# zzuiekongning/MGDT-YOLO

Measured on AMD Instinct MI355X. Metric: images/sec @640x640 bs=32 per GPU, detection forward + NMS (whole job: 1 GPU(s)), higher is better.
Workload: dtype bf16; 1 GPU; mspa_c2f_gd_yolov8-n (MSPA-C2f + GD neck + Detect, nc=80) 640x640 inference, batch 32/GPU: forward + decode + NMS(conf 0.25, iou 0.7), hipGraph replay, 4 batches in flight (one captured graph per resident batch, replayed round-robin on 4 streams); global_batch=32, parallelism=replicas x1 (batch-sharded, no data-path collective), rccl_ranks=1, input=bfloat16 NCHW images, 8 different batches resident in HBM (600 MiB) cycled, detections_last_step=9600, weights=seeded random init (no checkpoints offline), batches_in_flight=4

## Files before the change

### include/mgdt.h

```cpp
#ifndef MGDT_H
#define MGDT_H
#include <stddef.h>
#include <stdint.h>

#ifdef __cplusplus
extern "C" {
#endif

typedef void* mgdt_stream;

typedef enum { MGDT_OK = 0, MGDT_BAD_SHAPE = -1, MGDT_BAD_DTYPE = -2, MGDT_LAUNCH_FAIL = -3, MGDT_BAD_ARG = -4,
               MGDT_WORKSPACE = -5 } mgdt_status;
typedef enum { MGDT_F32 = 0, MGDT_BF16 = 1, MGDT_U8 = 2  } mgdt_dtype;
typedef enum { MGDT_ACT_NONE = 0, MGDT_ACT_SILU = 1, MGDT_ACT_RELU = 2, MGDT_ACT_GELU = 3 } mgdt_act;

typedef struct {
  void* p;
  int32_t n, h, w, c;
  int64_t sn, sh, sw, sc;
} mgdt_view;

const char* mgdt_last_error(void);
const char* mgdt_version(void);

// ... 33 lines not shown
size_t mgdt_cnx_mlp_packed_bytes(int c, int dtype);
int mgdt_cnx_mlp_pack(const float* w1, const float* b1, const float* w2, const float* b2, int c, void* packed, int dtype, mgdt_stream s);
size_t mgdt_cnx_mlp_workspace_bytes(int n, int h, int w, int c);
int mgdt_cnx_mlp_fwd(const mgdt_view* t, const mgdt_view* res, const void* packed, const float* gamma, const float* beta, void* ws,
                     const mgdt_view* y, int dtype, mgdt_stream s);

int mgdt_cnx_block_supported(int n, int h, int w, int c, int dtype);
size_t mgdt_cnx_block_workspace_bytes(int n, int h, int w, int c);
int mgdt_cnx_block_geometry(int h, int w, int c, int* out);
int mgdt_cnx_block_fwd(const mgdt_view* x, const float* dw_w49c, const float* dw_b, const float* ln_w, const float* ln_b, float eps, const void* packed,
                       const float* gamma, const float* beta, const void* tail_w, const float* tail_b, int tail_act, void* ws, size_t ws_bytes,
                       const mgdt_view* y, int dtype, mgdt_stream s);

size_t mgdt_stem2_packed_bytes(void);
int mgdt_stem2_pack(const float* w_folded, void* packed, mgdt_stream s);
int mgdt_stem2_fwd(const mgdt_view* x, int x_dtype, const void* packed0, const float* bias0, const void* packed1, const float* bias1,
                   const mgdt_view* y, mgdt_stream s);
int mgdt_stem2_geometry(int n, int h, int w, int cu_count, int* out);
int mgdt_stem2_route(const mgdt_view* x, int x_dtype, const mgdt_view* y, int cu_count, int* out);

int mgdt_detect_tail_supported(int c2, int c3, int nc, int reg_max, int dtype);
int mgdt_detect_tail_fwd(const mgdt_view* tb, const mgdt_view* tc, const void* wb, const float* bb, const void* wc, const float* bc, int nc,
                         float stride, int a_off, int a_total, const mgdt_view* feat, float* y, unsigned long long* best_keys,
                         const void* wb3, const float* bb3, mgdt_stream s);
int mgdt_detect_tail_aug_fwd(const mgdt_view* tb, const mgdt_view* tc, const void* wb, const float* bb, const void* wc, const float* bc, int nc,
                             float stride, int a_off, int a_total, const mgdt_view* feat, float* y, unsigned long long* best_keys,
                             const void* wb3, const float* bb3, float aug_scale, int aug_flip, float aug_img_w, mgdt_stream s);

int mgdt_scale_img_fwd(const mgdt_view* x, int x_dtype, int flip, int hs, int ws, float pad, const mgdt_view* y, int y_dtype, mgdt_stream s);

int mgdt_csp_block_supported(int mode, int cin, int cout, int wd, int nbtl, int h, int w, int dtype);
int mgdt_csp_block_tiles(int mode, int n, int cin, int cout, int wd, int nbtl, int h, int w, int* geom8);
int mgdt_csp_block_fwd(int mode, const mgdt_view* x, const void* front, const float* front_bias, const void* const* mid,
                       const float* const* mid_bias, int nbtl, int shortcut, const void* back, const float* back_bias, int wd, int act,
                       const mgdt_view* y, float* pool, int dtype, mgdt_stream s);

size_t mgdt_pw_chain_packed_bytes(int wd, int dtype);
int mgdt_pw_chain_pack(int idx, const float* w_oi, const float* conv_bias, const float* bn_gamma, const float* bn_beta, const float* bn_mean,
                       const float* bn_var, float bn_eps, int wd, int dtype, void* packed, mgdt_stream s);
int mgdt_pw_chain3_fwd(const mgdt_view* x, const void* packed, int wd, int act, const mgdt_view* y, int dtype, mgdt_stream s);

int mgdt_conv1x1_inject_supported(int cin, int cout, int h, int w, int hg, int wg, int dtype);
int mgdt_conv1x1_inject_fwd(const mgdt_view* x, const void* packed_w, const float* bias, const mgdt_view* ga, const mgdt_view* gf,
                            const mgdt_view* y, int dtype, mgdt_stream s);

int mgdt_conv1x1_inject_conv_supported(int cin, int cmid, int cout2, int h, int w, int hg, int wg, int dtype);
int mgdt_conv1x1_inject_conv_fwd(const mgdt_view* x, const void* packed_w, const float* bias, const mgdt_view* ga, const mgdt_view* gf,
                                 const mgdt_view* gsrc, const void* packed_wg, const float* bias_g, int cmid,
                                 const void* packed_w2, const float* bias2, int act2, const mgdt_view* y2, int dtype, mgdt_stream s);

int mgdt_laf_fuse_supported(int c0, int oc, int oc2, int h, int w, int h2, int w2, int act1, int act2, int dtype);
int mgdt_laf_fuse_fwd(const mgdt_view* p0, const mgdt_view* x1, const mgdt_view* x2, const void* packed_w1, const float* bias1, int act1,
                      const void* packed_w2, const float* bias2, int act2, const mgdt_view* y, int dtype, mgdt_stream s);

size_t mgdt_groupnorm_workspace_bytes(int n, int c);
int mgdt_groupnorm_fwd(const mgdt_view* x, const float* gamma, const float* beta, int groups, float eps, int act, void* ws, const mgdt_view* y,
                       int dtype, mgdt_stream s);
int mgdt_tood_layer_attn_fwd(const float* sums, int n, int c, int hw, const float* w1, const float* b1, const float* w2, const float* b2, int hid,
                             int stacked, float* scale, mgdt_stream s);
int mgdt_dcnv2_fwd(const mgdt_view* x, const mgdt_view* offset_mask, const float* w_gemm, const float* bias, const mgdt_view* y, int dtype,
                   mgdt_stream s);
int mgdt_dcnv2_mfma_fwd(const mgdt_view* x, const mgdt_view* offset_mask, const void* packed_w, const mgdt_view* y, int dtype, mgdt_stream s);
int mgdt_pixel_gate_fwd(const mgdt_view* x, const mgdt_view* gate, const mgdt_view* y, int dtype, mgdt_stream s);

int mgdt_conv_pack_direct(const float* w_oihw, const float* conv_bias, const float* bn_gamma, const float* bn_beta,
                          const float* bn_mean, const float* bn_var, float bn_eps, int cin_g, int cout, int k,
                          float* w_out, float* bias_out, mgdt_stream s);
int mgdt_conv2d_direct_fwd(const mgdt_view* x, int x_dtype, const float* w_gemm, const float* bias, int k, int stride,
                           int groups, int act, const mgdt_view* y, int dtype, mgdt_stream s);
enum { MGDT_DIRECT_STEM = 0, MGDT_DIRECT_GENERIC = 1, MGDT_DIRECT_REFUSED = 2 };
int mgdt_conv2d_direct_route(const mgdt_view* x, int x_dtype, const mgdt_view* y, int dtype, int k, int stride, int groups, int* out);

#define MGDT_SPR_SPLITS 16
int mgdt_spr_pool_fwd(const mgdt_view* x, float* pooled, int dtype, mgdt_stream s);
int mgdt_spr_attn_fwd(const float* pooled, const float* fc1_w, const float* fc1_b, const float* fc2_w,
                      const float* fc2_b, int n, int c, int groups, int h, int w, int softmax, float* attn, mgdt_stream s);
int mgdt_scale_channels_fwd(const mgdt_view* x, const float* attn, const mgdt_view* y, int dtype, mgdt_stream s);
int mgdt_spr_attn_scale_fwd(const float* pooled, int nsplit, int tiles_x, int tiles_y, const float* fc1_w, const float* fc1_b, const float* fc2_w, const float* fc2_b, int groups,
                            const mgdt_view* x, const mgdt_view* y, const mgdt_view* pool_a, const mgdt_view* pool_b, int dtype, mgdt_stream s);

int mgdt_sppf_pool_fwd(const mgdt_view* x, const mgdt_view* y1, const mgdt_view* y2, const mgdt_view* y3, int dtype,
                       mgdt_stream s);

int mgdt_adaptive_avgpool_fwd(const mgdt_view* x, const mgdt_view* y, int dtype, mgdt_stream s);
int mgdt_bilinear_fwd(const mgdt_view* x, const mgdt_view* y, int dtype, mgdt_stream s);
int mgdt_nearest_fwd(const mgdt_view* x, const mgdt_view* y, int dtype, mgdt_stream s);
int mgdt_copy_fwd(const mgdt_view* x, int x_dtype, const mgdt_view* y, int y_dtype, mgdt_stream s);
int mgdt_image_pad4_fwd(const mgdt_view* x, int x_dtype, const mgdt_view* y, int y_dtype, mgdt_stream s);

int mgdt_space_to_depth2_channels(int c, int y_dtype);
int mgdt_conv_pack_stem6(const float* w6, const float* conv_bias, const float* bn_gamma, const float* bn_beta, const float* bn_mean, const float* bn_var,
                         float bn_eps, int c6, int cout, int dtype, void* packed_out, float* bias_out, mgdt_stream s);
int mgdt_space_to_depth2_fwd(const mgdt_view* x, int x_dtype, const mgdt_view* y, int y_dtype, mgdt_stream s);
int mgdt_stem6_wgrad_unpack(const float* dw3, int cout, int cin, int cp, float* dw6, mgdt_stream s);

#define MGDT_GRN_SPLITS 8
int mgdt_dwconv7_ln_fwd(const mgdt_view* x, const float* dw_w, const float* dw_b, const float* ln_w, const float* ln_b,
                        float eps, const mgdt_view* y, int dtype, mgdt_stream s);
int mgdt_grn_stats_fwd(const mgdt_view* t, const float* gamma, float* ws, float* scale, int dtype, mgdt_stream s);
enum { MGDT_DW_ROW8 = 0, MGDT_DW_ROW10 = 1, MGDT_DW_GENERIC = 2 };
int mgdt_dwconv7_ln_route(int n, int h, int w, int c, int dtype, int* out);

int mgdt_inject_fwd(const mgdt_view* local, const mgdt_view* ga, const mgdt_view* gf, const mgdt_view* y, int dtype,
                    mgdt_stream s);

int mgdt_detect_decode_fwd(const mgdt_view* feat, int reg_max, int nc, float stride, int a_off, int a_total, float* y,
// ... 227 lines not shown
```

### mgdt_yolo_amd/_lib.py

```python
import ctypes as C
import os

_HERE = os.path.dirname(os.path.abspath(__file__))
LIB_PATH = os.environ.get('MGDT_LIB') or os.path.join(_HERE, 'csrc', 'libmgdt_hip.so')

F32, BF16 = 0, 1
ACT_NONE, ACT_SILU, ACT_RELU, ACT_GELU = 0, 1, 2, 3
SPR_SPLITS = 16
GRN_SPLITS = 8


class View(C.Structure):
    _fields_ = [('p', C.c_void_p), ('n', C.c_int32), ('h', C.c_int32), ('w', C.c_int32), ('c', C.c_int32),
                ('sn', C.c_int64), ('sh', C.c_int64), ('sw', C.c_int64), ('sc', C.c_int64)]


VP = C.POINTER(View)
_vp, _i, _f, _sz, _l = C.c_void_p, C.c_int, C.c_float, C.c_size_t, C.c_long

class PackDesc(C.Structure):
    _fields_ = [('w', C.c_void_p), ('conv_bias', C.c_void_p), ('bn_gamma', C.c_void_p), ('bn_beta', C.c_void_p), ('bn_mean', C.c_void_p), ('bn_var', C.c_void_p),
                ('bn_eps', C.c_float), ('cin', C.c_int32), ('cout', C.c_int32), ('k', C.c_int32), ('dtype', C.c_int32), ('mode', C.c_int32),
                ('packed', C.c_void_p), ('bias_out', C.c_void_p)]

# ... 10 lines not shown
ROUTE_X2, ROUTE_IN_SCALE, ROUTE_IN_SHIFT, ROUTE_R1, ROUTE_R2, ROUTE_FP8 = 1, 2, 4, 8, 16, 32
ROUTE_IGEMM, ROUTE_LDS3X3 = 0, 1
DIRECT_STEM, DIRECT_GENERIC, DIRECT_REFUSED = 0, 1, 2

PROTOTYPES = {
    'mgdt_last_error': (C.c_char_p, []),
    'mgdt_version': (C.c_char_p, []),
    'mgdt_conv_packed_bytes': (_sz, [_i, _i, _i, _i]),
    'mgdt_conv_pack': (_i, [_vp, _vp, _vp, _vp, _vp, _vp, _f, _i, _i, _i, _i, _vp, _vp, _vp]),
    'mgdt_conv2d_fwd': (_i, [VP, VP, _vp, _vp, _vp, _vp, _i, _i, _i, VP, VP, VP, _i, _vp]),
    'mgdt_conv_packed_bytes_fp8': (_sz, [_i, _i, _i]),
    'mgdt_conv_pack_fp8': (_i, [_vp, _vp, _vp, _vp, _vp, _vp, _f, _i, _i, _i, _f, _vp, _vp, _vp, _vp]),
    'mgdt_conv2d_fp8_fwd': (_i, [VP, VP, _vp, _vp, _vp, _vp, _vp, _f, _i, _i, _i, VP, VP, VP, _vp]),
    'mgdt_conv2d_route': (_i, [VP, VP, _i, _i, _i, _i, _i, C.POINTER(ConvRoute)]),
    'mgdt_conv_pack_batch': (_i, [_vp, _i, _vp]),
    'mgdt_conv2d_phase_fwd': (_i, [VP, _vp, _vp, _i, VP, VP, VP, _i, _vp]),
    'mgdt_conv_wgrad_splits': (_i, [_i, _i, _i]),
    'mgdt_wgrad_final_batch': (_i, [_vp, _i, _vp]),
    'mgdt_conv_pack_dgrad': (_i, [_vp, _i, _i, _i, _i, _i, _vp, _vp, _vp]),
    'mgdt_conv_pack_direct': (_i, [_vp, _vp, _vp, _vp, _vp, _vp, _f, _i, _i, _i, _vp, _vp, _vp]),
    'mgdt_conv2d_direct_fwd': (_i, [VP, _i, _vp, _vp, _i, _i, _i, _i, VP, _i, _vp]),
    'mgdt_conv2d_direct_route': (_i, [VP, _i, VP, _i, _i, _i, _i, C.POINTER(C.c_int)]),
    'mgdt_spr_pool_fwd': (_i, [VP, _vp, _i, _vp]),
    'mgdt_spr_attn_fwd': (_i, [_vp, _vp, _vp, _vp, _vp, _i, _i, _i, _i, _i, _i, _vp, _vp]),
    'mgdt_scale_channels_fwd': (_i, [VP, _vp, VP, _i, _vp]),
    'mgdt_sppf_pool_fwd': (_i, [VP, VP, VP, VP, _i, _vp]),
    'mgdt_adaptive_avgpool_fwd': (_i, [VP, VP, _i, _vp]),
    'mgdt_bilinear_fwd': (_i, [VP, VP, _i, _vp]),
    'mgdt_nearest_fwd': (_i, [VP, VP, _i, _vp]),
    'mgdt_copy_fwd': (_i, [VP, _i, VP, _i, _vp]),
    'mgdt_image_pad4_fwd': (_i, [VP, _i, VP, _i, _vp]),
    'mgdt_space_to_depth2_channels': (_i, [_i, _i]),
    'mgdt_space_to_depth2_fwd': (_i, [VP, _i, VP, _i, _vp]),
    'mgdt_conv_pack_stem6': (_i, [_vp, _vp, _vp, _vp, _vp, _vp, _f, _i, _i, _i, _vp, _vp, _vp]),
    'mgdt_stem6_wgrad_unpack': (_i, [_vp, _i, _i, _i, _vp, _vp]),
    'mgdt_dwconv7_ln_fwd': (_i, [VP, _vp, _vp, _vp, _vp, _f, VP, _i, _vp]),
    'mgdt_cnx_mlp_packed_bytes': (_sz, [_i, _i]),
    'mgdt_cnx_mlp_pack': (_i, [_vp, _vp, _vp, _vp, _i, _vp, _i, _vp]),
    'mgdt_cnx_mlp_workspace_bytes': (_sz, [_i, _i, _i, _i]),
    'mgdt_cnx_mlp_fwd': (_i, [VP, VP, _vp, _vp, _vp, _vp, VP, _i, _vp]),
    'mgdt_cnx_block_supported': (_i, [_i, _i, _i, _i, _i]),
    'mgdt_cnx_block_workspace_bytes': (_sz, [_i, _i, _i, _i]),
    'mgdt_cnx_block_geometry': (_i, [_i, _i, _i, C.POINTER(C.c_int)]),
    'mgdt_cnx_block_fwd': (_i, [VP, _vp, _vp, _vp, _vp, _f, _vp, _vp, _vp, _vp, _vp, _i, _vp, _sz, VP, _i, _vp]),
    'mgdt_pw_chain_packed_bytes': (_sz, [_i, _i]),
    'mgdt_pw_chain_pack': (_i, [_i, _vp, _vp, _vp, _vp, _vp, _vp, _f, _i, _i, _vp, _vp]),
    'mgdt_pw_chain3_fwd': (_i, [VP, _vp, _i, _i, VP, _i, _vp]),
    'mgdt_conv1x1_inject_supported': (_i, [_i, _i, _i, _i, _i, _i, _i]),
    'mgdt_conv1x1_inject_fwd': (_i, [VP, _vp, _vp, VP, VP, VP, _i, _vp]),
    'mgdt_conv1x1_inject_conv_supported': (_i, [_i, _i, _i, _i, _i, _i, _i, _i]),
    'mgdt_conv1x1_inject_conv_fwd': (_i, [VP, _vp, _vp, VP, VP, VP, _vp, _vp, _i, _vp, _vp, _i, VP, _i, _vp]),
    'mgdt_laf_fuse_supported': (_i, [_i, _i, _i, _i, _i, _i, _i, _i, _i, _i]),
    'mgdt_laf_fuse_fwd': (_i, [VP, VP, VP, _vp, _vp, _i, _vp, _vp, _i, VP, _i, _vp]),
    'mgdt_spr_attn_scale_fwd': (_i, [_vp, _i, _i, _i, _vp, _vp, _vp, _vp, _i, VP, VP, VP, VP, _i, _vp]),
    'mgdt_stem2_packed_bytes': (_sz, []),
    'mgdt_stem2_pack': (_i, [_vp, _vp, _vp]),
    'mgdt_stem2_fwd': (_i, [VP, _i, _vp, _vp, _vp, _vp, VP, _vp]),
    'mgdt_stem2_geometry': (_i, [_i, _i, _i, _i, C.POINTER(C.c_int)]),
    'mgdt_stem2_route': (_i, [VP, _i, VP, _i, C.POINTER(C.c_int)]),
    'mgdt_detect_tail_supported': (_i, [_i, _i, _i, _i, _i]),
    'mgdt_detect_tail_fwd': (_i, [VP, VP, _vp, _vp, _vp, _vp, _i, _f, _i, _i, VP, _vp, _vp, _vp, _vp, _vp]),
    'mgdt_detect_tail_aug_fwd': (_i, [VP, VP, _vp, _vp, _vp, _vp, _i, _f, _i, _i, VP, _vp, _vp, _vp, _vp, _f, _i, _f, _vp]),
    'mgdt_scale_img_fwd': (_i, [VP, _i, _i, _i, _i, _f, VP, _i, _vp]),
    'mgdt_csp_block_supported': (_i, [_i, _i, _i, _i, _i, _i, _i, _i]),
    'mgdt_csp_block_tiles': (_i, [_i, _i, _i, _i, _i, _i, _i, _i, _vp]),
    'mgdt_csp_block_fwd': (_i, [_i, VP, _vp, _vp, _vp, _vp, _i, _i, _vp, _vp, _i, _i, VP, _vp, _i, _vp]),
    'mgdt_groupnorm_workspace_bytes': (_sz, [_i, _i]),
    'mgdt_groupnorm_fwd': (_i, [VP, _vp, _vp, _i, _f, _i, _vp, VP, _i, _vp]),
    'mgdt_tood_layer_attn_fwd': (_i, [_vp, _i, _i, _i, _vp, _vp, _vp, _vp, _i, _i, _vp, _vp]),
    'mgdt_dcnv2_fwd': (_i, [VP, VP, _vp, _vp, VP, _i, _vp]),
    'mgdt_dcnv2_mfma_fwd': (_i, [VP, VP, _vp, VP, _i, _vp]),
    'mgdt_pixel_gate_fwd': (_i, [VP, VP, VP, _i, _vp]),
    'mgdt_gn_affine_workspace_bytes': (_sz, [_i, _i, _i]),
    'mgdt_gn_affine': (_i, [VP, _vp, _vp, _i, _f, _vp, _vp, _vp, _vp, _vp, _i, _vp]),
    'mgdt_nc_affine_act_bwd': (_i, [VP, VP, _vp, _vp, _i, VP, _i, _vp]),
    'mgdt_gn_act_grad': (_i, [VP, VP, _vp, _vp, _vp, _i, _i, VP, _i, _vp]),
    'mgdt_gn_bwd_workspace_bytes': (_sz, [_i, _i]),
    'mgdt_gn_bwd_coef': (_i, [VP, VP, _vp, _vp, _i, _vp, _vp, _vp, _vp, _vp, _i, _vp, _i, _vp]),
    'mgdt_nc_axpby': (_i, [VP, _vp, VP, _vp, _vp, VP, _i, _vp]),
    'mgdt_pixel_gate_bwd': (_i, [VP, VP, VP, VP, VP, _i, _vp]),
    'mgdt_tood_layer_attn_bwd_workspace_bytes': (_sz, [_i, _i, _i, _i]),
    'mgdt_tood_layer_attn_bwd': (_i, [_vp, _vp, _i, _i, _i, _vp, _vp, _vp, _vp, _i, _i, _vp, _vp, _vp, _vp, _vp, _i, _vp, _vp]),
    'mgdt_dcn_im2col': (_i, [VP, VP, VP, _i, _vp]),
    'mgdt_dcn_col2im_bwd': (_i, [VP, VP, VP, _vp, VP, _i, _vp]),
    'mgdt_val_match_fwd': (_i, [_vp, _vp, _i, _i, _vp, _vp, _i, _vp, _i, _vp, _vp]),
    'mgdt_grn_stats_fwd': (_i, [VP, _vp, _vp, _vp, _i, _vp]),
    'mgdt_dwconv7_ln_route': (_i, [_i, _i, _i, _i, _i, C.POINTER(C.c_int)]),
    'mgdt_inject_fwd': (_i, [VP, VP, VP, VP, _i, _vp]),
    'mgdt_detect_decode_fwd': (_i, [VP, _i, _i, _f, _i, _i, _vp, _i, _vp]),
    'mgdt_detect_decode_aug_fwd': (_i, [VP, _i, _i, _f, _i, _i, _vp, _vp, _f, _i, _f, _i, _vp]),
    'mgdt_detect_loss_workspace_bytes': (_sz, [_i, _i, _i]),
    'mgdt_detect_loss_fwd': (_i, [_vp, _vp, _i, _i, _i, _vp, _i, _i, _f, _f, _f, _vp, _vp, _vp, _vp, _vp, _sz, _i, _vp]),
    'mgdt_detect_loss_fwd_dev': (_i, [_vp, _vp, _i, _i, _i, _vp, _i, _vp, _f, _f, _f, _vp, _vp, _vp, _vp, _vp, _sz, _i, _vp]),
    'mgdt_detect_loss_bwd': (_i, [_vp, _vp, _vp, _i, _i, _i, _vp, _i, _f, _f, _f, _f, _vp, _vp, _sz, _i, _vp]),
    'mgdt_reduce_workspace_bytes': (_sz, [_i]),
    'mgdt_bn_stats_fwd': (_i, [VP, _f, _f, _vp, _vp, _vp, _vp, _vp, _i, _vp]),
    'mgdt_bn_act_fwd': (_i, [VP, _vp, _vp, _vp, _vp, _i, VP, VP, VP, _i, _vp]),
    'mgdt_bn_act_bwd': (_i, [VP, VP, _vp, _vp, _vp, _vp, _i, _vp, _vp, VP, _vp, _i, _vp]),
    'mgdt_conv_dgrad': (_i, [VP, _vp, _i, _i, VP, _i, _i, _vp]),
    'mgdt_gconv_dgrad': (_i, [VP, _vp, _i, _i, _i, VP, _i, _i, _vp]),
    'mgdt_gconv_wgrad_workspace_bytes': (_sz, [_i, _i, _i, _i]),
    'mgdt_gconv_wgrad': (_i, [VP, VP, _i, _i, _i, _vp, _i, _vp, _i, _vp]),
    'mgdt_conv_wgrad_workspace_bytes': (_sz, [_i, _i, _i]),
    'mgdt_conv_wgrad': (_i, [VP, VP, VP, _i, _i, _vp, _vp, _i, _vp, _i, _vp]),
    'mgdt_add_fwd': (_i, [VP, VP, VP, _i, _vp]),
    'mgdt_maxpool5_bwd': (_i, [VP, VP, _vp, _i, _vp]),
# ... 106 lines not shown
```

### mgdt_yolo_amd/nn/modules/block.py

```python
import torch
import torch.nn as nn

from ... import ops
from .conv import Conv, HipModule, act_code
from .convnextv2 import ConvNeXtV2_Block
from .spr_module import SPRModule

__all__ = ('DFL', 'SPP', 'SPPF', 'C2f', 'C3', 'MSPA_C2f', 'Bottleneck', 'SimFusion_4in', 'SimFusion_3in', 'IFM', 'h_sigmoid',
           'InjectionMultiSum_Auto_pool', 'Upsample', 'Proto')


def _plain_block(first, last, bottlenecks):
    def conv_ok(c, k):
        return (isinstance(c, Conv) and c.plain_affine() and c.conv.kernel_size == (k, k) and c.conv.stride == (1, 1) and c.conv.groups == 1
                and act_code(c.act) == a0)
    try:
        a0 = act_code(first.act)
    except RuntimeError:
        return False
    if a0 != ops.ACT_SILU:
        return False
    if not (conv_ok(first, 1) and conv_ok(last, 1)) or len(bottlenecks) == 0:
        return False
    return all(isinstance(m, Bottleneck) and conv_ok(m.cv1, 3) and conv_ok(m.cv2, 3) and m.add == bottlenecks[0].add
# ... 214 lines not shown
                   and c.conv.out_channels == self.inwidth and act_code(c.act) == act_code(cs[0].act) for c in cs)

    def _packed_chain(self, dtype):
        cs = list(self.convs)[:3]
        tens = [t for c in cs for t in c.affine_tensors()]
        return self._cached(('chain', dtype), tens, lambda: ops.PackedPwChain([(c.conv.weight, c.conv.bias, c.bn_tuple()) for c in cs], dtype))

    def backward(self, g):
        out, attn, part, xshape = self._ctx.pop()
        wd, s, n = self.inwidth, self.nums, self.btnk_nums
        at = self.attention
        dattn = ops.nc_reduce(g, out)
        prms = (at.fc1.weight, at.fc1.bias, at.fc2.weight, at.fc2.bias)
        gb = [ops.grad_buf(p) for p in prms]
        chained = all(t.is_contiguous() and t.dtype == torch.float32 for t in gb) and all(
            a.untyped_storage().data_ptr() == b.untyped_storage().data_ptr() and a.storage_offset() + a.numel() == b.storage_offset() for a, b in zip(gb, gb[1:]))
        pg_out = gb[0].new_empty(0).set_(gb[0].untyped_storage(), gb[0].storage_offset(), (sum(t.numel() for t in gb),)) if chained else None
        gout, pg = ops.spr_bwd(g, part, attn, dattn, at.fc1.weight, at.fc1.bias, at.fc2.weight, at.fc2.bias, s, out=pg_out)
        if not chained:
            o = 0
            for prm, t in zip(prms, gb):
                t.copy_(pg[o:o + t.numel()].view_as(prm))
                o += t.numel()
        gcat = self.convs[s - 1].backward(gout)
        gx = ops.new_act(xshape[0], xshape[1], xshape[2], xshape[3], g.dtype, g.device)
        sl = lambda t, i: t[:, i * wd:(i + 1) * wd]
        for j in reversed(range(n)):
            if j > 0:
                self.bottleneck[j].backward(sl(gcat, s - 1 + j), acc_into=sl(gcat, s - 2 + j))
                continue
            gin = self.bottleneck[j].backward(sl(gcat, s - 1 + j))
            dst = sl(gcat, s - 2 + j)
            ops.add(dst, gin, out=dst)
            ops.copy(gin, sl(gx, s - 1))
        for i in reversed(range(1, s - 1)):
            gi = self.convs[i].backward(sl(gcat, i), dx_out=sl(gx, i))
            dst = sl(gcat, i - 1)
            ops.add(dst, gi, out=dst)
        self.convs[0].backward(sl(gcat, 0), dx_out=sl(gx, 0))
        return gx


class SPPF(HipModule):

    def __init__(self, c1, c2, k=5):
        super().__init__()
        if k != 5:
            raise RuntimeError('SPPF: k=5 is what the YAMLs use and what the fused pooling kernel implements')
        c_ = c1 // 2
        self.cv1 = Conv(c1, c_, 1, 1)
        self.cv2 = Conv(c_ * 4, c2, 1, 1)
        self.m = nn.MaxPool2d(kernel_size=k, stride=1, padding=k // 2)

    def forward(self, x):
        b, _, h, w = x.shape
        c_ = self.cv1.conv.out_channels
        train = self.training and hasattr(self.cv1, 'bn')
        cat = ops.new_act(b, 4 * c_, h, w, self.cv1.out_dtype(x), x.device)
        (self.cv1.train_fwd if train else self.cv1.run)(x, out=cat[:, :c_])
        ops.sppf_pools(cat[:, :c_], cat[:, c_:2 * c_], cat[:, 2 * c_:3 * c_], cat[:, 3 * c_:])
        if train:
            self._cat = cat if ops.ctx_enabled() else None
        return (self.cv2.train_fwd if train else self.cv2.run)(cat)

    def backward(self, g):
        c_ = self.cv1.conv.out_channels
        cat, self._cat = self._cat, None
        gcat = self.cv2.backward(g)
        sl = lambda t, i: t[:, i * c_:(i + 1) * c_]
        g2 = ops.add(sl(gcat, 2), ops.maxpool5_bwd(sl(cat, 2), sl(gcat, 3)))
        g1 = ops.add(sl(gcat, 1), ops.maxpool5_bwd(sl(cat, 1), g2))
        g0 = ops.add(sl(gcat, 0), ops.maxpool5_bwd(sl(cat, 0), g1))
        return self.cv1.backward(g0)


class SPP(SPPF):

    def __init__(self, c1, c2, k=(5, 9, 13)):
        if tuple(k) != (5, 9, 13):
            raise RuntimeError(f'SPP: k=(5, 9, 13) is what the YAMLs use and what the pooling kernels implement, got {tuple(k)}')
        super().__init__(c1, c2, 5)
        self.m = nn.ModuleList([nn.MaxPool2d(kernel_size=x, stride=1, padding=x // 2) for x in k])

    def backward(self, g):
        c_ = self.cv1.conv.out_channels
        cat, self._cat = self._cat, None
        gcat = self.cv2.backward(g)
        sl = lambda t, i: t[:, i * c_:(i + 1) * c_]
        g0 = ops.add(sl(gcat, 0), ops.spp_pool_bwd(sl(cat, 0), sl(gcat, 1), sl(gcat, 2), sl(gcat, 3)))
        return self.cv1.backward(g0)


class Proto(HipModule):

    def __init__(self, c1, c_=256, c2=32):
        super().__init__()
        self.cv1 = Conv(c1, c_, k=3)
        self.upsample = nn.ConvTranspose2d(c_, c_, 2, 2, 0, bias=True)
        self.cv2 = Conv(c_, c_, k=3)
        self.cv3 = Conv(c_, c2)

    def run_upsample(self, x):
        up = self.upsample
        ops.check_deconv2x2(up.kernel_size, up.stride, up.padding, up.groups, up.output_padding, up.dilation)
        if up.bias is None:
            raise RuntimeError('Proto.upsample is built with its bias (block.py:63)')
        dt = self.out_dtype(x)
        pk = self._cached(('deconv', dt), [up.weight, up.bias], lambda: ops.PackedDeconv2x2(up.weight, up.bias, dt))
        return ops.deconv2x2(x, pk)

# ... 270 lines not shown
```

### mgdt_yolo_amd/ops.py

```python
import ctypes as C
import os

import numpy as np
import torch

from . import _lib as L
from ._lib import ACT_GELU, ACT_NONE, ACT_RELU, ACT_SILU, BF16, F32, View

U8 = 2
_DT = {torch.float32: F32, torch.bfloat16: BF16}


def dtype_code(dt):
    try:
        return _DT[dt]
    except KeyError:
        raise RuntimeError(f'mgdt_yolo_amd computes in float32 or bfloat16, not {dt}') from None


def _need_gpu(t):
    if not t.is_cuda:
        raise RuntimeError('mgdt_yolo_amd runs on MI355X (HIP) only: got a CPU tensor and there is no CPU/PyTorch fallback')


# ... 652 lines not shown


def conv1x1_inject_conv_supported(x, cmid, cout2, ga, dtype):
    return bool(FUSED_INJECT and FUSED_INJECT_CONV and x.dtype == dtype and ga.dtype == dtype and is_nhwc(x) and is_nhwc(ga) and
                L.lib().mgdt_conv1x1_inject_conv_supported(x.shape[1], cmid, cout2, x.shape[2], x.shape[3], ga.shape[2], ga.shape[3], dtype_code(dtype)))


def conv1x1_inject_conv(x, pk, ga, gf, pk2, act2, out, gsrc=None, pkg=None):
    b, _, h, w = x.shape
    _same(x, ga, gf, gsrc, out)
    if _PROF is not None:
        _META['conv1x1_inject_conv_fwd'] = dict(shape=(b, pk.cin, h, w, pk2.cout, 1, 1), flops=2.0 * b * h * w * (pk.cout * pk.cin + pk2.cout * pk2.cin),
                                                bytes=float(b * h * w * (pk.cin + pk2.cout) * x.element_size() + (2 * ga.numel() * ga.element_size() if gsrc is None else gsrc.numel() * 2)))
    _launch('conv1x1_inject_conv_fwd', 'mgdt_conv1x1_inject_conv_fwd', vp(x), ptr(pk.w), ptr(pk.bias), vp(ga), vp(gf), vp(gsrc), None if pkg is None else ptr(pkg.w),
            None if pkg is None else ptr(pkg.bias), pk.cout, ptr(pk2.w), ptr(pk2.bias), int(act2), vp(out), dtype_code(pk.dtype), stream())
    return out


FUSED_INJECT_CONV = True
FUSED_INJECT_GCONV = True


def conv1x1_inject(x, pk, ga, gf, out=None):
    b, _, h, w = x.shape
    if out is None:
        out = new_act(b, pk.cout, h, w, pk.dtype, x.device)
    if _PROF is not None:
        _META['conv1x1_inject_fwd'] = dict(shape=(b, pk.cin, h, w, pk.cout, 1, 1), flops=2.0 * b * h * w * pk.cout * pk.cin,
                                           bytes=float(b * h * w * (pk.cin + pk.cout) * x.element_size() + 2 * ga.numel() * ga.element_size()))
    _launch('conv1x1_inject_fwd', 'mgdt_conv1x1_inject_fwd', vp(x), ptr(pk.w), ptr(pk.bias), vp(ga), vp(gf), vp(out), dtype_code(pk.dtype), stream())
    return out


FUSED_LAF = True


def laf_fuse_supported(p0, x1, x2, oc2, act1, act2, dtype):
    return bool(FUSED_LAF and p0.dtype == dtype and x1.dtype == dtype and x2.dtype == dtype and is_nhwc(p0) and is_nhwc(x1) and is_nhwc(x2) and
                x2.shape[1] == x1.shape[1] and p0.shape[0] == x1.shape[0] == x2.shape[0] and p0.shape[2:] == x1.shape[2:] and
                all(t.stride(0) % 8 == 0 and t.stride(2) % 8 == 0 and t.stride(3) % 8 == 0 and t.data_ptr() % 16 == 0 for t in (p0, x1, x2)) and
                L.lib().mgdt_laf_fuse_supported(p0.shape[1], x1.shape[1], oc2, x1.shape[2], x1.shape[3], x2.shape[2], x2.shape[3], int(act1), int(act2),
                                                dtype_code(dtype)))


def laf_fuse(p0, x1, x2, pk1, act1, pk2, act2, out=None):
    b, oc, h, w = x1.shape
    if out is None:
        out = new_act(b, pk2.cout, h, w, pk2.dtype, x1.device)
    _same(p0, x1, x2, out)
    if _PROF is not None:
        _META['laf_fuse_fwd'] = dict(shape=(b, pk1.cin, h, w, pk2.cout, 1, 1), flops=2.0 * b * h * w * (pk1.cout * pk1.cin + pk2.cout * pk2.cin),
                                     bytes=float((b * h * w * (pk1.cin + oc + pk2.cout) + x2.numel()) * x1.element_size()))
    _launch('laf_fuse_fwd', 'mgdt_laf_fuse_fwd', vp(p0), vp(x1), vp(x2), ptr(pk1.w), ptr(pk1.bias), int(act1), ptr(pk2.w), ptr(pk2.bias), int(act2), vp(out),
            dtype_code(pk2.dtype), stream())
    return out


def groupnorm(x, gamma, beta, groups, eps, act, out=None):
    b, c = x.shape[:2]
    out = like(x) if out is None else out
    ws = torch.empty(L.lib().mgdt_groupnorm_workspace_bytes(b, c), dtype=torch.uint8, device=x.device)
    _launch('groupnorm_fwd', 'mgdt_groupnorm_fwd', vp(x), ptr(gamma), ptr(beta), groups, float(eps), act, ptr(ws), vp(out), dtype_code(x.dtype), stream())
    return out


def tood_layer_attn(feat, w1, b1, w2, b2, stacked, sums=None):
    b, c, h, w = feat.shape
    sums = nc_reduce(feat) if sums is None else sums
    scale = torch.empty(b, c, dtype=torch.float32, device=feat.device)
    _launch('tood_layer_attn_fwd', 'mgdt_tood_layer_attn_fwd', ptr(sums), b, c, h * w, ptr(w1), ptr(b1), ptr(w2), ptr(b2), w1.shape[0], stacked, ptr(scale), stream())
    return scale


def dcnv2(x, offset_mask, w_gemm, bias, cout):
    b, _, h, w = x.shape
    out = new_act(b, cout, h, w, x.dtype, x.device)
    _launch('dcnv2_fwd', 'mgdt_dcnv2_fwd', vp(x), vp(offset_mask), ptr(w_gemm), ptr(bias), vp(out), dtype_code(x.dtype), stream())
    return out


def dcnv2_mfma(x, offset_mask, pk, out=None):
    b, _, h, w = x.shape
    out = new_act(b, pk.cout, h, w, x.dtype, x.device) if out is None else out
    _same(x, offset_mask, out)
    _launch('dcnv2_mfma_fwd', 'mgdt_dcnv2_mfma_fwd', vp(x), vp(offset_mask), ptr(pk.w), vp(out), dtype_code(x.dtype), stream())
    return out


def pixel_gate(x, gate, out=None):
    out = like(x) if out is None else out
    _launch('pixel_gate_fwd', 'mgdt_pixel_gate_fwd', vp(x), vp(gate), vp(out), dtype_code(x.dtype), stream())
    return out


def _gn_affine(y, gamma, beta, groups, eps):
    b, c, h, w = y.shape
    dev = y.device
    A, B = torch.empty(b, c, dtype=torch.float32, device=dev), torch.empty(b, c, dtype=torch.float32, device=dev)
    mean, rstd = torch.empty(b, groups, dtype=torch.float32, device=dev), torch.empty(b, groups, dtype=torch.float32, device=dev)
    ws = torch.empty(L.lib().mgdt_gn_affine_workspace_bytes(b, c, groups), dtype=torch.uint8, device=dev)
    _launch('gn_affine', 'mgdt_gn_affine', vp(y), ptr(gamma), ptr(beta), groups, float(eps), ptr(mean), ptr(rstd), ptr(A), ptr(B), ptr(ws), dtype_code(y.dtype), stream())
    return A, B, mean, rstd, ws[ws.numel() - b * groups * 16:].view(torch.float64).view(b, groups, 2)


def gn_affine(y, gamma, beta, groups, eps):
    return _gn_affine(y, gamma, beta, groups, eps)[:4]
# ... 1631 lines not shown
```

Before: 42410 images/sec.

## Fuse SPPF cv1, cascaded max-pools and cv2 into one LDS-resident kernel

Adds a HIP kernel that runs the whole SPPF block per spatial tile with a 6-pixel halo. It computes cv1 with MFMA into LDS, applies the three cascaded 5x5 max-pools as separable row/column passes in LDS using an order-preserving bf16 key, and accumulates cv2 over the four concat slices before writing only the final output. The aim is to remove the HBM round trips for the 4*c_ concat tensor and the separate pool and conv launches. In exchange, halo pixels are recomputed for every tile and LDS use is large, which limits how many workgroups fit per CU.

After: 43210 images/sec (median of 6 runs). +1.9%, better.

```diff
diff --git a/include/mgdt.h b/include/mgdt.h
--- a/include/mgdt.h
+++ b/include/mgdt.h
@@ -109,6 +109,10 @@
 int mgdt_laf_fuse_supported(int c0, int oc, int oc2, int h, int w, int h2, int w2, int act1, int act2, int dtype);
 int mgdt_laf_fuse_fwd(const mgdt_view* p0, const mgdt_view* x1, const mgdt_view* x2, const void* packed_w1, const float* bias1, int act1,
                       const void* packed_w2, const float* bias2, int act2, const mgdt_view* y, int dtype, mgdt_stream s);
+
+int mgdt_sppf_fuse_supported(int c1, int cm, int c2, int h, int w, int act1, int act2, int dtype);
+int mgdt_sppf_fuse_fwd(const mgdt_view* x, const void* packed_w1, const float* bias1, int act1, const void* packed_w2, const float* bias2, int act2,
+                       const mgdt_view* y, int dtype, mgdt_stream s);
 
 size_t mgdt_groupnorm_workspace_bytes(int n, int c);
 int mgdt_groupnorm_fwd(const mgdt_view* x, const float* gamma, const float* beta, int groups, float eps, int act, void* ws, const mgdt_view* y,
diff --git a/mgdt_yolo_amd/_lib.py b/mgdt_yolo_amd/_lib.py
--- a/mgdt_yolo_amd/_lib.py
+++ b/mgdt_yolo_amd/_lib.py
@@ -86,6 +86,8 @@
     'mgdt_conv1x1_inject_conv_fwd': (_i, [VP, _vp, _vp, VP, VP, VP, _vp, _vp, _i, _vp, _vp, _i, VP, _i, _vp]),
     'mgdt_laf_fuse_supported': (_i, [_i, _i, _i, _i, _i, _i, _i, _i, _i, _i]),
     'mgdt_laf_fuse_fwd': (_i, [VP, VP, VP, _vp, _vp, _i, _vp, _vp, _i, VP, _i, _vp]),
+    'mgdt_sppf_fuse_supported': (_i, [_i, _i, _i, _i, _i, _i, _i, _i]),
+    'mgdt_sppf_fuse_fwd': (_i, [VP, _vp, _vp, _i, _vp, _vp, _i, VP, _i, _vp]),
     'mgdt_spr_attn_scale_fwd': (_i, [_vp, _i, _i, _i, _vp, _vp, _vp, _vp, _i, VP, VP, VP, VP, _i, _vp]),
     'mgdt_stem2_packed_bytes': (_sz, []),
     'mgdt_stem2_pack': (_i, [_vp, _vp, _vp]),
diff --git a/mgdt_yolo_amd/csrc/sppf_fused.hip b/mgdt_yolo_amd/csrc/sppf_fused.hip
--- /dev/null
+++ b/mgdt_yolo_amd/csrc/sppf_fused.hip
@@ -0,0 +1,309 @@
+#include <algorithm>
+
+#include "conv_igemm_kernel.h"
+
+struct SppfArgs {
+  const char* x; int xsn, xsh, xsw; uint32_t x_bytes;
+  const char* y; int ysn, ysh, ysw; uint32_t y_bytes;
+  const char* w1; const float* b1; const char* w2; const float* b2;
+  int H, W, T, tiles_x, tiles_img, act1, act2;
+  int a_bytes;
+  unsigned long long* dbg;
+};
+
+constexpr int SPPF_THREADS = 512, SPPF_CPAD = 8;
+constexpr int SPPF_TILES[] = {10, 8, 6, 5, 4, 3, 2, 1};
+constexpr int SPPF_STATIC = 2048;
+constexpr int SPPF_LDS = 160 * 1024 - SPPF_STATIC;
+
+typedef __attribute__((ext_vector_type(2))) float sppf_f32x2;
+typedef __attribute__((ext_vector_type(2))) __bf16 sppf_bf16x2;
+typedef __attribute__((ext_vector_type(8))) short sppf_i16x8;
+typedef __attribute__((ext_vector_type(4))) unsigned int sppf_u32x4;
+typedef __attribute__((__vector_size__(2 * sizeof(unsigned int)))) unsigned int sppf_u32x2v;
+__device__ __forceinline__ uint32_t sppf_pk_bf16(float lo, float hi) {
+  return __builtin_bit_cast(uint32_t, __builtin_convertvector(sppf_f32x2{lo, hi}, sppf_bf16x2));
+}
+__device__ __forceinline__ uint32_t sppf_key(uint32_t v) { return v ^ (((v >> 15) & 0x00010001u) * 0x7fffu); }
+__device__ __forceinline__ sppf_u32x4 sppf_key4(sppf_u32x4 v) { return sppf_u32x4{sppf_key(v[0]), sppf_key(v[1]), sppf_key(v[2]), sppf_key(v[3])}; }
+__device__ __forceinline__ sppf_u32x4 sppf_kmax(sppf_u32x4 p, sppf_u32x4 q) {
+  return __builtin_bit_cast(sppf_u32x4, __builtin_elementwise_max(__builtin_bit_cast(sppf_i16x8, p), __builtin_bit_cast(sppf_i16x8, q)));
+}
+__device__ __forceinline__ float sppf_nan_pos(float v) { return v != v ? __uint_as_float(0x7fc00000u) : v; }
+__device__ __forceinline__ int sppf_clamp(int v, int hi) { return min(max(v, 0), hi); }
+
+template <int KC1, int NB2>
+__global__ __launch_bounds__(SPPF_THREADS) void sppf_fuse_kernel(const SppfArgs a) {
+  typedef bf16x8 frag;
+  constexpr int NB1 = KC1, KCM = KC1 / 2, CQ = 2 * KC1;
+  constexpr int RS = (NB1 * 16 + SPPF_CPAD) * 2;
+  constexpr int W1V = KC1 * NB1 * 64;
+  constexpr int CW = NB2 % 4 == 0 ? 4 : 2, NBW = NB2 / CW;
+  constexpr int PW = 8 / CW, MT2 = (7 + PW - 1) / PW;
+  static_assert((NB1 + NB2) * 16 * sizeof(float) <= SPPF_STATIC, "the bias vectors outgrow their share of the 160 KiB");
+  static_assert(KC1 % 2 == 0 && MT2 * PW >= 7, "whole K chunks per concat slot; seven pixel groups of a 10 x 10 tile");
+  extern __shared__ __attribute__((aligned(16))) char sppf_sm[];
+  __shared__ __attribute__((aligned(16))) float bl1[NB1 * 16];
+  __shared__ __attribute__((aligned(16))) float bl2[NB2 * 16];
+  char* const A = sppf_sm;
+  char* const B = sppf_sm + a.a_bytes;
+  const int tid = threadIdx.x, lane = tid & 63;
+  const int wave = __builtin_amdgcn_readfirstlane(tid >> 6);
+  const int r = lane & 15, g = lane >> 4;
+  unsigned long long* const dbgw = (a.dbg && tid == 0) ? a.dbg + (size_t)blockIdx.x * 8 : nullptr;
+  if (dbgw) dbgw[0] = wall_clock64();
+
+  const int n = (int)blockIdx.x / a.tiles_img, tile = (int)blockIdx.x - n * a.tiles_img;
+  const int tyi = tile / a.tiles_x, txi = tile - tyi * a.tiles_x;
+  const int H = a.H, W = a.W;
+  const int y0 = tyi * a.T, x0 = txi * a.T, th = min(a.T, H - y0), tw = min(a.T, W - x0);
+  const int ry0 = max(y0 - 6, 0), ry1 = min(y0 + th + 6, H), rx0 = max(x0 - 6, 0), rx1 = min(x0 + tw + 6, W);
+  const int RH = ry1 - ry0, RW = rx1 - rx0, RP = RH * RW, NG1 = (RP + 15) >> 4;
+  const int uy0 = max(y0 - 4, 0), uy1 = min(y0 + th + 4, H), ux0 = max(x0 - 4, 0), ux1 = min(x0 + tw + 4, W), UW = ux1 - ux0;
+  const int vy0 = max(y0 - 2, 0), vy1 = min(y0 + th + 2, H), vx0 = max(x0 - 2, 0), vx1 = min(x0 + tw + 2, W), VW = vx1 - vx0;
+
+  const __amdgpu_buffer_rsrc_t xrs = __builtin_amdgcn_make_buffer_rsrc((void*)a.x, 0, a.x_bytes, 0x00020000);
+  const __amdgpu_buffer_rsrc_t yrs = __builtin_amdgcn_make_buffer_rsrc((void*)a.y, 0, a.y_bytes, 0x00020000);
+
+  auto request = [&](int p, frag(&P)[2][KC1]) __attribute__((always_inline)) {
+#pragma unroll
+    for (int mt = 0; mt < 2; ++mt) {
+      const int rp = (2 * p + mt) * 16 + r;
+      const bool pv = rp < RP;
+      const int rr = pv ? rp / RW : 0, rc = pv ? rp - rr * RW : 0;
+      const int off = pv ? n * a.xsn + (ry0 + rr) * a.xsh + (rx0 + rc) * a.xsw : MGDT_OOB;
+#pragma unroll
+      for (int kc = 0; kc < KC1; ++kc)
+        P[mt][kc] = __builtin_bit_cast(frag, __builtin_amdgcn_raw_buffer_load_b128(xrs, (uint32_t)(off + (kc * 4 + g) * 16), 0, 0));
+    }
+  };
+  frag P[2][KC1];
+  int p = wave;
+  request(p, P);
+
+  const int cw = wave % CW, pw = wave / CW;
+  const char* const w2lane = a.w2 + ((size_t)(cw * NBW) * 64 + lane) * 16;
+  frag Wc[KCM][NBW];
+  auto request_w2 = [&](int s) __attribute__((always_inline)) {
+#pragma unroll
+    for (int kc = 0; kc < KCM; ++kc)
+#pragma unroll
+      for (int nb = 0; nb < NBW; ++nb) Wc[kc][nb] = *(const frag*)(w2lane + (size_t)((s * KCM + kc) * NB2 + nb) * 1024);
+  };
+
+  {
+    constexpr int N1 = (W1V + SPPF_THREADS - 1) / SPPF_THREADS;
+#pragma unroll
+    for (int u = 0; u < N1; ++u) {
+      const int i = tid + u * SPPF_THREADS;
+      if (W1V % SPPF_THREADS == 0 || i < W1V) ((uint4*)B)[i] = ((const uint4*)a.w1)[i];
+    }
+    if (tid < NB1 * 16) bl1[tid] = a.b1[tid];
+    if (tid < NB2 * 16) bl2[tid] = a.b2[tid];
+  }
+  __syncthreads();
+  if (dbgw) dbgw[1] = wall_clock64();
+  request_w2(0);
+
+
+  auto cv1_blocks = [&](auto actf) __attribute__((always_inline)) {
+    const char* const w1lane = B + lane * 16;
+    while (2 * p < NG1) {
+      char* const dst = A + (2 * p * 16 + r) * RS + 8 * g;
+      const bool second = 2 * p + 1 < NG1;
+#pragma unroll 1
+      for (int nb = 0; nb < NB1; ++nb) {
+        f32x4 acc0 = *(const f32x4*)(&bl1[nb * 16 + 4 * g]), acc1 = acc0;
+#pragma unroll
+        for (int kc = 0; kc < KC1; ++kc) {
+          const frag Wf = *(const frag*)(w1lane + (kc * NB1 + nb) * 1024);
+          acc0 = mma(Wf, P[0][kc], acc0);
+          acc1 = mma(Wf, P[1][kc], acc1);
+        }
+        *(uint2*)(dst + nb * 32) = make_uint2(sppf_key(sppf_pk_bf16(sppf_nan_pos(actf(acc0[0])), sppf_nan_pos(actf(acc0[1])))),
+                                              sppf_key(sppf_pk_bf16(sppf_nan_pos(actf(acc0[2])), sppf_nan_pos(actf(acc0[3])))));
+        if (second)
+          *(uint2*)(dst + 16 * RS + nb * 32) = make_uint2(sppf_key(sppf_pk_bf16(sppf_nan_pos(actf(acc1[0])), sppf_nan_pos(actf(acc1[1])))),
+                                                          sppf_key(sppf_pk_bf16(sppf_nan_pos(actf(acc1[2])), sppf_nan_pos(actf(acc1[3])))));
+      }
+      p += 8;
+      if (2 * p < NG1) request(p, P);
+    }
+  };
+  switch (a.act1) {
+    case MGDT_ACT_SILU: cv1_blocks([](float v) { return v * fast_sigmoid(v); }); break;
+    case MGDT_ACT_RELU: cv1_blocks([](float v) { return fmaxf(v, 0.f); }); break;
+    default: cv1_blocks([](float v) { return v; }); break;
+  }
+  __syncthreads();
+  if (dbgw) dbgw[2] = wall_clock64();
+
+  int aoff[MT2], voff[MT2], yo[MT2];
+#pragma unroll
+  for (int mt = 0; mt < MT2; ++mt) {
+    const int t = (pw + PW * mt) * 16 + r;
+    const bool pv = t < th * tw;
+    const int tt = pv ? t : 0, tr = tt / tw, tc = tt - tr * tw;
+    const int row = y0 + tr, col = x0 + tc;
+    aoff[mt] = ((row - ry0) * RW + (col - rx0)) * RS + 16 * g;
+    voff[mt] = ((row - vy0) * VW + (col - vx0)) * RS + 16 * g;
+    yo[mt] = pv ? n * a.ysn + row * a.ysh + col * a.ysw + 8 * g : MGDT_OOB;
+  }
+  f32x4 acc2[NBW][MT2];
+#pragma unroll
+  for (int nb = 0; nb < NBW; ++nb) {
+    const f32x4 b = *(const f32x4*)(&bl2[(cw * NBW + nb) * 16 + 4 * g]);
+#pragma unroll
+    for (int mt = 0; mt < MT2; ++mt) acc2[nb][mt] = b;
+  }
+
+  auto max4 = [&](const char* src, int sy0, int sx0, int SW, int rw, int c, int cq) __attribute__((always_inline)) {
+    const int ra = (sppf_clamp(rw - 2, H - 1) - sy0) * SW - sx0, rb = (sppf_clamp(rw + 2, H - 1) - sy0) * SW - sx0;
+    const int ca = sppf_clamp(c - 2, W - 1), cb = sppf_clamp(c + 2, W - 1);
+    const char* const base = src + cq * 16;
+    return sppf_kmax(sppf_kmax(*(const sppf_u32x4*)(base + (ra + ca) * RS), *(const sppf_u32x4*)(base + (ra + cb) * RS)),
+                     sppf_kmax(*(const sppf_u32x4*)(base + (rb + ca) * RS), *(const sppf_u32x4*)(base + (rb + cb) * RS)));
+  };
+
+#pragma unroll 1
+  for (int s = 0; s < 4; ++s) {
+    const char* const plane = s == 2 ? B : A;
+#pragma unroll
+    for (int kc = 0; kc < KCM; ++kc) {
+      frag Bf[MT2];
+#pragma unroll
+      for (int mt = 0; mt < MT2; ++mt) Bf[mt] = __builtin_bit_cast(frag, sppf_key4(*(const sppf_u32x4*)(plane + (s == 2 ? voff[mt] : aoff[mt]) + kc * 64)));
+#pragma unroll
+      for (int nb = 0; nb < NBW; ++nb)
+#pragma unroll
+        for (int mt = 0; mt < MT2; ++mt) acc2[nb][mt] = mma(Wc[kc][nb], Bf[mt], acc2[nb][mt]);
+      __builtin_amdgcn_sched_barrier(0);
+    }
+    if (s == 3) break;
+    request_w2(s + 1);
+    __builtin_amdgcn_sched_barrier(0);
+    if (s == 0) {
+      for (int i = tid; i < RH * UW * CQ; i += SPPF_THREADS) {
+        const int cq = i % CQ, px = i / CQ, rr = px / UW, cc = px - rr * UW, c = ux0 + cc;
+        const int rowi = rr * RW - rx0;
+        const char* const base = A + cq * 16;
+        sppf_u32x4 m = *(const sppf_u32x4*)(base + (rowi + c) * RS);
+#pragma unroll
+        for (int d = -2; d <= 2; ++d)
+          if (d) m = sppf_kmax(m, *(const sppf_u32x4*)(base + (rowi + sppf_clamp(c + d, W - 1)) * RS));
+        *(sppf_u32x4*)(B + px * RS + cq * 16) = m;
+      }
+      __syncthreads();
+      if (dbgw) dbgw[3] = wall_clock64();
+      for (int i = tid; i < (uy1 - uy0) * UW * CQ; i += SPPF_THREADS) {
+        const int cq = i % CQ, px = i / CQ, rr = px / UW, cc = px - rr * UW, rw = uy0 + rr;
+        const char* const base = B + cq * 16;
+        sppf_u32x4 m = *(const sppf_u32x4*)(base + (px + (uy0 - ry0) * UW) * RS);
+#pragma unroll
+        for (int d = -2; d <= 2; ++d)
+          if (d) m = sppf_kmax(m, *(const sppf_u32x4*)(base + ((sppf_clamp(rw + d, H - 1) - ry0) * UW + cc) * RS));
+        *(sppf_u32x4*)(A + ((rw - ry0) * RW + (ux0 + cc - rx0)) * RS + cq * 16) = m;
+      }
+    } else if (s == 1) {
+      for (int i = tid; i < (vy1 - vy0) * VW * CQ; i += SPPF_THREADS) {
+        const int cq = i % CQ, px = i / CQ, rr = px / VW, cc = px - rr * VW;
+        *(sppf_u32x4*)(B + px * RS + cq * 16) = max4(A, ry0, rx0, RW, vy0 + rr, vx0 + cc, cq);
+      }
+    } else {
+      for (int i = tid; i < th * tw * CQ; i += SPPF_THREADS) {
+        const int cq = i % CQ, px = i / CQ, rr = px / tw, cc = px - rr * tw;
+        *(sppf_u32x4*)(A + ((y0 + rr - ry0) * RW + (x0 + cc - rx0)) * RS + cq * 16) = max4(B, vy0, vx0, VW, y0 + rr, x0 + cc, cq);
+      }
+    }
+    __syncthreads();
+    if (dbgw) dbgw[4 + s] = wall_clock64();
+  }
+
+  auto epilogue = [&](auto actf) __attribute__((always_inline)) {
+#pragma unroll
+    for (int mt = 0; mt < MT2; ++mt)
+#pragma unroll
+      for (int nb = 0; nb < NBW; ++nb) {
+        const f32x4 c = acc2[nb][mt];
+        const sppf_u32x2v o = {sppf_pk_bf16(actf(c[0]), actf(c[1])), sppf_pk_bf16(actf(c[2]), actf(c[3]))};
+        __builtin_amdgcn_raw_buffer_store_b64(o, yrs, (uint32_t)(yo[mt] + (cw * NBW + nb) * 32), 0, 0);
+      }
+  };
+  switch (a.act2) {
+    case MGDT_ACT_SILU: epilogue([](float v) { return v * fast_sigmoid(v); }); break;
+    case MGDT_ACT_RELU: epilogue([](float v) { return fmaxf(v, 0.f); }); break;
+    default: epilogue([](float v) { return v; }); break;
+  }
+  if (dbgw) dbgw[7] = wall_clock64();
+}
+
+static bool sppf_act_ok(int act) { return act == MGDT_ACT_NONE || act == MGDT_ACT_SILU || act == MGDT_ACT_RELU; }
+
+static int sppf_extent(int size, int t, int halo) {
+  int m = 0;
+  for (int o = 0; o < size; o += t) m = std::max(m, std::min(o + std::min(t, size - o) + halo, size) - std::max(o - halo, 0));
+  return m;
+}
+static bool sppf_plan(int cm, int h, int w, int* T, int* a_bytes, int* lds) {
+  const int RS = (cm + SPPF_CPAD) * 2, panel = (2 * cm / 32) * (cm / 16) * 1024;
+  for (int t : SPPF_TILES) {
+    const int rh = sppf_extent(h, t, 6), rw = sppf_extent(w, t, 6), uw = sppf_extent(w, t, 4);
+    const long ab = (long)cdiv((long)rh * rw, 16) * 16 * RS, bb = std::max((long)panel, (long)rh * uw * RS);
+    if (ab + bb > SPPF_LDS) continue;
+    *T = t; *a_bytes = (int)ab; *lds = (int)(ab + bb);
+    return true;
+  }
+  return false;
+}
+
+extern "C" int mgdt_sppf_fuse_supported(int c1, int cm, int c2, int h, int w, int act1, int act2, int dtype) {
+  if (dtype != MGDT_BF16 || c1 != 2 * cm || h < 1 || w < 1 || h > 4096 || w > 4096 || !sppf_act_ok(act1) || !sppf_act_ok(act2)) return 0;
+  if (!((c1 == 64 && (c2 == 64 || c2 == 96)) || (c1 == 256 && c2 == 256))) return 0;
+  int T, ab, lds;
+  return sppf_plan(cm, h, w, &T, &ab, &lds) ? 1 : 0;
+}
+
+template <int KC1, int NB2>
+static int sppf_launch(const SppfArgs& a, int grid, int lds, hipStream_t st) {
+  if (int rc = lds_optin<sppf_fuse_kernel<KC1, NB2>>("sppf_fuse", SPPF_LDS)) return rc;
+  static StampBuf stamps;
+  SppfArgs b = a;
+  const bool dbg = knob_set("MGDT_SPPF_DBG");
+  if (dbg && !stamps.ensure((size_t)grid * 8)) MGDT_FAIL(MGDT_WORKSPACE, "sppf_fuse: no memory for the MGDT_SPPF_DBG stamps");
+  b.dbg = dbg ? stamps.p : nullptr;
+  sppf_fuse_kernel<KC1, NB2><<<grid, SPPF_THREADS, lds, st>>>(b);
+  MGDT_CHECK_LAUNCH("sppf_fuse_fwd");
+  if (dbg) {
+    const std::vector<unsigned long long> h = stamps.read((size_t)grid * 8, st);
+    unsigned long long t0 = ~0ull, t7 = 0; double ph[7] = {0, 0, 0, 0, 0, 0, 0};
+    for (int i = 0; i < grid; ++i) { t0 = std::min(t0, h[i * 8]); t7 = std::max(t7, h[i * 8 + 7]); for (int j = 0; j < 7; ++j) ph[j] += (double)(h[i * 8 + j + 1] - h[i * 8 + j]); }
+    fprintf(stderr, "sppf_fuse x10ns: %d WGs, span %llu; avg per WG: load+stage %.0f cv1 %.0f x0+rowmax %.0f colmax %.0f y1+Y2 %.0f y2+y3 %.0f y3+store %.0f\n", grid, t7 - t0,
+            ph[0] / grid, ph[1] / grid, ph[2] / grid, ph[3] / grid, ph[4] / grid, ph[5] / grid, ph[6] / grid);
+  }
+  return MGDT_OK;
+}
+
+extern "C" int mgdt_sppf_fuse_fwd(const mgdt_view* x, const void* packed_w1, const float* bias1, int act1, const void* packed_w2, const float* bias2,
+                                  int act2, const mgdt_view* y, int dtype, mgdt_stream s) {
+  if (!view_ok(x) || !view_ok(y) || !packed_w1 || !bias1 || !packed_w2 || !bias2) MGDT_FAIL(MGDT_BAD_ARG, "sppf_fuse: null/empty argument");
+  if (!mgdt_sppf_fuse_supported(x->c, x->c / 2, y->c, y->h, y->w, act1, act2, dtype))
+    MGDT_FAIL(MGDT_BAD_SHAPE, "sppf_fuse: shapes/dtype/activations not covered (see mgdt_sppf_fuse_supported)");
+  if (x->n != y->n || x->h != y->h || x->w != y->w) MGDT_FAIL(MGDT_BAD_SHAPE, "sppf_fuse: x and y must share n, h, w");
+  SppfArgs a;
+  memset(&a, 0, sizeof(a));
+  const ViewPolicy vx = {8, true, 0, 0, false}, vy = {4, true, 0, 0, false};
+  if (!bind_view(x, 2, vx, &a.x, &a.xsn, &a.xsh, &a.xsw, &a.x_bytes) || !bind_view(y, 2, vy, &a.y, &a.ysn, &a.ysh, &a.ysw, &a.y_bytes))
+    MGDT_FAIL(MGDT_BAD_SHAPE, "sppf_fuse: views must be NHWC (sc == 1), x 16-byte and y 8-byte aligned, and < 2 GiB");
+  int lds = 0;
+  if (!sppf_plan(x->c / 2, y->h, y->w, &a.T, &a.a_bytes, &lds)) MGDT_FAIL(MGDT_BAD_SHAPE, "sppf_fuse: no tile fits LDS");
+  a.w1 = (const char*)packed_w1; a.b1 = bias1; a.w2 = (const char*)packed_w2; a.b2 = bias2; a.act1 = act1; a.act2 = act2;
+  a.H = y->h; a.W = y->w; a.tiles_x = cdiv(a.W, a.T); a.tiles_img = a.tiles_x * cdiv(a.H, a.T);
+  const long grid = (long)y->n * a.tiles_img;
+  if (grid >= 0x7fffffffL) MGDT_FAIL(MGDT_BAD_SHAPE, "sppf_fuse: too many tiles");
+  hipStream_t st = (hipStream_t)s;
+  const int kc1 = x->c / 32, nb2 = y->c / 16;
+#define SPPF_CASE(K, N) if (kc1 == K && nb2 == N) return sppf_launch<K, N>(a, (int)grid, lds, st);
+  SPPF_CASE(2, 4) SPPF_CASE(2, 6) SPPF_CASE(8, 16)
+#undef SPPF_CASE
+  MGDT_FAIL(MGDT_BAD_SHAPE, "sppf_fuse: no kernel for kc1=%d nb2=%d", kc1, nb2);
+}
diff --git a/mgdt_yolo_amd/nn/modules/block.py b/mgdt_yolo_amd/nn/modules/block.py
--- a/mgdt_yolo_amd/nn/modules/block.py
+++ b/mgdt_yolo_amd/nn/modules/block.py
@@ -290,10 +290,30 @@
         self.cv2 = Conv(c_ * 4, c2, 1, 1)
         self.m = nn.MaxPool2d(kernel_size=k, stride=1, padding=k // 2)
 
+    def _fused_route(self, x):
+        c1, c2 = self.cv1, self.cv2
+        dt = torch.bfloat16
+        if self.training or not ops.FUSED_SPPF or x.dtype != dt or ops.Q8_CALIB is not None or not isinstance(c1, Conv) or not isinstance(c2, Conv):
+            return None
+        for c in (c1, c2):
+            if (not c.plain_affine() or c.conv.kernel_size != (1, 1) or c.conv.stride != (1, 1) or c.conv.padding != (0, 0) or c.conv.groups != 1
+                    or not isinstance(c.act, (nn.Identity, nn.SiLU, nn.ReLU)) or c.__dict__.get('_q8') or c.out_dtype(x) != dt):
+                return None
+        if self.__dict__.get('_q8') or self._forward_hooks or c1._forward_hooks or c2._forward_hooks:
+            return None
+        cm, co = c1.conv.out_channels, c2.conv.out_channels
+        if (c1.conv.in_channels != x.shape[1] or c2.conv.in_channels != 4 * cm or not ops.conv_can_mfma(x, x.shape[1], cm, 1, 1, 1, dt)
+                or not ops.sppf_fuse_supported(x, cm, co, act_code(c1.act), act_code(c2.act), dt)):
+            return None
+        return lambda: ops.sppf_fuse(x, c1.packed(dt, direct=False), act_code(c1.act), c2.packed(dt, direct=False), act_code(c2.act))
+
     def forward(self, x):
         b, _, h, w = x.shape
         c_ = self.cv1.conv.out_channels
         train = self.training and hasattr(self.cv1, 'bn')
+        fused = self._fused_route(x)
+        if fused is not None:
+            return fused()
         cat = ops.new_act(b, 4 * c_, h, w, self.cv1.out_dtype(x), x.device)
         (self.cv1.train_fwd if train else self.cv1.run)(x, out=cat[:, :c_])
         ops.sppf_pools(cat[:, :c_], cat[:, c_:2 * c_], cat[:, 2 * c_:3 * c_], cat[:, 3 * c_:])
diff --git a/mgdt_yolo_amd/ops.py b/mgdt_yolo_amd/ops.py
--- a/mgdt_yolo_amd/ops.py
+++ b/mgdt_yolo_amd/ops.py
@@ -728,6 +728,28 @@
         _META['laf_fuse_fwd'] = dict(shape=(b, pk1.cin, h, w, pk2.cout, 1, 1), flops=2.0 * b * h * w * (pk1.cout * pk1.cin + pk2.cout * pk2.cin),
                                      bytes=float((b * h * w * (pk1.cin + oc + pk2.cout) + x2.numel()) * x1.element_size()))
     _launch('laf_fuse_fwd', 'mgdt_laf_fuse_fwd', vp(p0), vp(x1), vp(x2), ptr(pk1.w), ptr(pk1.bias), int(act1), ptr(pk2.w), ptr(pk2.bias), int(act2), vp(out),
+            dtype_code(pk2.dtype), stream())
+    return out
+
+
+FUSED_SPPF = True
+
+
+def sppf_fuse_supported(x, cm, c2, act1, act2, dtype):
+    return bool(FUSED_SPPF and x.dtype == dtype and is_nhwc(x) and
+                x.stride(0) % 8 == 0 and x.stride(2) % 8 == 0 and x.stride(3) % 8 == 0 and x.data_ptr() % 16 == 0 and
+                L.lib().mgdt_sppf_fuse_supported(x.shape[1], cm, c2, x.shape[2], x.shape[3], int(act1), int(act2), dtype_code(dtype)))
+
+
+def sppf_fuse(x, pk1, act1, pk2, act2, out=None):
+    b, _, h, w = x.shape
+    if out is None:
+        out = new_act(b, pk2.cout, h, w, pk2.dtype, x.device)
+    _same(x, out)
+    if _PROF is not None:
+        _META['sppf_fuse_fwd'] = dict(shape=(b, pk1.cin, h, w, pk2.cout, 1, 1), flops=2.0 * b * h * w * (pk1.cout * pk1.cin + pk2.cout * pk2.cin),
+                                      bytes=float(b * h * w * (pk1.cin + pk2.cout) * x.element_size()))
+    _launch('sppf_fuse_fwd', 'mgdt_sppf_fuse_fwd', vp(x), ptr(pk1.w), ptr(pk1.bias), int(act1), ptr(pk2.w), ptr(pk2.bias), int(act2), vp(out),
             dtype_code(pk2.dtype), stream())
     return out
 
```
